# uwoseis/zephyr

Hardware: AMD Instinct MI355X
Metric: wavefields/sec (freq x source solves/s) on 1024^2 grid (higher is better)
Workload: dtype f64

## Files before the change

### include/helm.h

```cpp
#ifndef HELM_H
#define HELM_H

#include <stddef.h>

#ifdef __cplusplus
extern "C" {
#endif

typedef struct helm_op helm_op;

enum { HELM_MINIZEPHYR = 0, HELM_EURUS = 1, HELM_3D = 2  };

enum {
    HELM_BICGSTAB = 0,
    HELM_CGNR = 1,
    HELM_AUTO = 2,
    HELM_MG = 3,
    HELM_DIRECT = 4
};

enum {
    HELM_OK = 0,
    HELM_ERR_ARG = -1,
    HELM_ERR_DEVICE = -2,
// ... 197 lines not shown
    int    pf_prio;
    int    mg3_keep;
    int    mg3_keep_levels;
    int    mg3_galerkin;
    int    mg3_depth_model;
    int    mg3_bt_f32;
    int    mg3_otf;
    int    mg3_f32;
    double mg3_omega;
    int    mg3_coarse;
    int    mg3_nd_leaf;
    int    mg3_bt_twist;
    double mg3_beta;
    double sync_spin_ms;
    int    sync_sleep_us;
    int    nd_fused_sep;
    int    nd_fused_sep_min;
} helm_tuning;
int helm_get_tuning(helm_tuning *out);
int helm_set_tuning(const helm_tuning *t);

int helm_direct_plan(int nz, int nx, int leaf, int *out, int cap);
int helm_direct_plan_front(int nz, int nx, int leaf, int node, long long *cells, int cap);
int helm_debug_zgemm(int device, int M, int N, int K, const double *alpha, const double *A, const double *B,
                     const double *beta, double *C, int batch);
int helm_debug_inverse(int device, int n, double *A, int batch);
int helm_debug_zgemm_bench(int device, int M, int N, int K, int batch, int variant, int reps, double *ms_out);
#define HELM_ZG_TABLE 1
#define HELM_ZG_MASKS 2
#define HELM_ZG_TM64  4
int helm_debug_zgemm_choice(int M, int N, int K, int batch, int nf_div, int force_tile, int force_slab, int have_handle, int mode, int report[5]);
typedef struct helm_zgemm_ex {
    int device, M, N, K, batch;
    int lda, ldb, ldc;
    long long sa, sb, sc;
    double alpha[2], beta[2];
    const double *A; long long a_len;
    double *B; long long b_len;
    double *C; long long c_len;
    int force_tile, force_slab;
    int xcd_map;
    int ntc;
    int zr0, zr1, zc0, zc1, sk0, sk1;
    int tm64, c_is_b;
    const int *tabB, *tabCi, *tabCo; long long tab_len;
    int tab_stride, offB, offCi, offCo;
// ... 53 lines not shown
```

### zephyr_amd/_lib.py

```python
import ctypes
import os
import numpy as np

_HERE = os.path.dirname(os.path.abspath(__file__))
LIB_PATH = os.path.join(_HERE, 'libhelm.so')

HELM_MINIZEPHYR, HELM_EURUS, HELM_3D = 0, 1, 2
HELM_BICGSTAB, HELM_CGNR, HELM_AUTO, HELM_MG, HELM_DIRECT = 0, 1, 2, 3, 4
HELM_RHS_NODE_MAJOR, HELM_OUT_NODE_MAJOR, HELM_NODE_MAJOR = 1, 2, 3
METHODS = {'bicgstab': HELM_BICGSTAB, 'cgnr': HELM_CGNR, 'auto': HELM_AUTO, 'mg': HELM_MG, 'direct': HELM_DIRECT}

ERRORS = {-1: 'HELM_ERR_ARG', -2: 'HELM_ERR_DEVICE', -3: 'HELM_ERR_STATE', -4: 'HELM_ERR_UNSUPPORTED', -5: 'HELM_ERR_PML'}


class HelmError(RuntimeError):
    def __init__(self, code, text):
        self.code = code
        RuntimeError.__init__(self, '%s: %s' % (ERRORS.get(code, code), text))


class SolveOpts(ctypes.Structure):
    _fields_ = [('method', ctypes.c_int), ('rtol', ctypes.c_double), ('maxit', ctypes.c_int),
                ('check_every', ctypes.c_int), ('batch', ctypes.c_int), ('flags', ctypes.c_int)]

# ... 9 lines not shown
                ('factor_ms', ctypes.c_double), ('gemm_ms', ctypes.c_double),
                ('gemm_launches', ctypes.c_longlong), ('gemm_flops', ctypes.c_double),
                ('gemm_big_ms', ctypes.c_double), ('gemm_big_launches', ctypes.c_longlong), ('gemm_big_flops', ctypes.c_double),
                ('gemm_bytes', ctypes.c_double), ('gemm_sol_ms', ctypes.c_double)]


class Tuning(ctypes.Structure):
    _fields_ = [('nd_leaf', ctypes.c_int), ('nd_ws_gb', ctypes.c_double), ('nd_sparse_rhs', ctypes.c_int), ('nd_stable', ctypes.c_int),
                ('nd_stable_thr', ctypes.c_double), ('nd_stable_safety', ctypes.c_double), ('nd_fused_leaf', ctypes.c_int),
                ('nd_fused_leaf_min', ctypes.c_int), ('nd_gjstep', ctypes.c_int), ('nd_gjstep_min', ctypes.c_int), ('nd_overlap', ctypes.c_int),
                ('nd_xcd_map', ctypes.c_int), ('nd_plans', ctypes.c_int), ('nd_direct_out', ctypes.c_int), ('nd_many', ctypes.c_int), ('nd_leaf_idle', ctypes.c_int), ('auto_direct', ctypes.c_int),
                ('auto_mg3', ctypes.c_int), ('prof_ext', ctypes.c_int), ('ws_slots', ctypes.c_int), ('pf_prio', ctypes.c_int),
                ('mg3_keep', ctypes.c_int), ('mg3_keep_levels', ctypes.c_int), ('mg3_galerkin', ctypes.c_int), ('mg3_depth_model', ctypes.c_int),
                ('mg3_bt_f32', ctypes.c_int), ('mg3_otf', ctypes.c_int), ('mg3_f32', ctypes.c_int), ('mg3_omega', ctypes.c_double),
                ('mg3_coarse', ctypes.c_int), ('mg3_nd_leaf', ctypes.c_int), ('mg3_bt_twist', ctypes.c_int), ('mg3_beta', ctypes.c_double), ('sync_spin_ms', ctypes.c_double), ('sync_sleep_us', ctypes.c_int),
                ('nd_fused_sep', ctypes.c_int), ('nd_fused_sep_min', ctypes.c_int)]


class RuntimeStats(ctypes.Structure):
    _fields_ = [('dev_allocs', ctypes.c_longlong), ('dev_alloc_bytes', ctypes.c_double), ('dev_alloc_ms', ctypes.c_double),
                ('host_allocs', ctypes.c_longlong), ('host_alloc_bytes', ctypes.c_double), ('host_alloc_ms', ctypes.c_double),
                ('events_created', ctypes.c_longlong), ('streams_created', ctypes.c_longlong),
                ('first_launches', ctypes.c_longlong), ('first_launch_ms', ctypes.c_double),
                ('kernels_registered', ctypes.c_longlong), ('kernels_resolved', ctypes.c_longlong), ('warm_ms', ctypes.c_double),
                ('dev_frees', ctypes.c_longlong), ('dev_free_ms', ctypes.c_double),
                ('sync_calls', ctypes.c_longlong), ('sync_ms', ctypes.c_double), ('slow_syncs', ctypes.c_longlong), ('worst_sync_ms', ctypes.c_double)]


class ZgemmEx(ctypes.Structure):
    _fields_ = [('device', ctypes.c_int), ('M', ctypes.c_int), ('N', ctypes.c_int), ('K', ctypes.c_int), ('batch', ctypes.c_int),
# ... 125 lines not shown
                                         ctypes.c_void_p, ctypes.c_longlong]),
    'helm_pack_c64_device': (ctypes.c_int, [ctypes.c_void_p, ctypes.c_void_p, ctypes.c_int, ctypes.c_longlong, ctypes.c_void_p, ctypes.c_void_p]),
    'helm_imaging_accumulate_c64_device': (ctypes.c_int, [ctypes.c_void_p, ctypes.c_void_p, ctypes.c_void_p, ctypes.c_void_p, ctypes.c_int,
                                                          ctypes.c_void_p, ctypes.c_void_p]),
    'helm_sample_rows_c64_device': (ctypes.c_int, [ctypes.c_void_p, ctypes.c_void_p, ctypes.c_void_p, ctypes.c_int, ctypes.c_longlong, ctypes.c_void_p,
                                                   ctypes.c_void_p, ctypes.c_void_p, ctypes.c_int, ctypes.c_longlong, ctypes.c_double, ctypes.c_double,
                                                   ctypes.c_double, ctypes.c_double, ctypes.c_void_p]),
    'helm_direct_plan': (ctypes.c_int, [ctypes.c_int, ctypes.c_int, ctypes.c_int, ctypes.c_void_p, ctypes.c_int]),
    'helm_direct_plan_front': (ctypes.c_int, [ctypes.c_int, ctypes.c_int, ctypes.c_int, ctypes.c_int, ctypes.c_void_p, ctypes.c_int]),
    'helm_mg3_axis': (ctypes.c_int, [ctypes.c_int, ctypes.c_int, ctypes.c_double, ctypes.c_double, ctypes.c_double, ctypes.c_double, ctypes.c_int,
                                     ctypes.c_void_p, ctypes.c_void_p, ctypes.c_void_p, ctypes.c_void_p, ctypes.c_void_p, ctypes.c_void_p, ctypes.c_void_p,
                                     ctypes.c_void_p]),
    'helm_debug_zgemm': (ctypes.c_int, [ctypes.c_int, ctypes.c_int, ctypes.c_int, ctypes.c_int, ctypes.c_void_p, ctypes.c_void_p,
                                        ctypes.c_void_p, ctypes.c_void_p, ctypes.c_void_p, ctypes.c_int]),
    'helm_debug_zgemm_choice': (ctypes.c_int, [ctypes.c_int] * 9 + [ctypes.POINTER(ctypes.c_int)]),
    'helm_debug_zgemm_ex': (ctypes.c_int, [ctypes.POINTER(ZgemmEx)]),
    'helm_debug_nm_stage': (ctypes.c_int, [ctypes.c_void_p]),
    'helm_debug_inverse': (ctypes.c_int, [ctypes.c_int, ctypes.c_int, ctypes.c_void_p, ctypes.c_int]),
    'helm_debug_zgemm_bench': (ctypes.c_int, [ctypes.c_int, ctypes.c_int, ctypes.c_int, ctypes.c_int, ctypes.c_int, ctypes.c_int, ctypes.c_int,
                                              ctypes.POINTER(ctypes.c_double)]),
    'helm_set_rhs_support': (ctypes.c_int, [ctypes.c_void_p, ctypes.c_void_p, ctypes.c_longlong, ctypes.c_int]),
    'helm_rhs_support_from_coo': (ctypes.c_int, [ctypes.c_void_p, ctypes.c_void_p, ctypes.c_void_p, ctypes.c_longlong, ctypes.c_void_p, ctypes.c_longlong, ctypes.c_int]),
    'helm_regrid_axis': (ctypes.c_int, [ctypes.c_int, ctypes.c_double, ctypes.c_int, ctypes.c_double, ctypes.c_void_p, ctypes.c_void_p, ctypes.c_int]),
    'helm_regrid_create': (ctypes.c_void_p, [ctypes.c_int, ctypes.c_int, ctypes.c_int, ctypes.c_double, ctypes.c_double, ctypes.c_int, ctypes.c_int,
                                             ctypes.c_double, ctypes.c_double, ctypes.c_double, ctypes.c_double]),
    'helm_regrid_destroy': (None, [ctypes.c_void_p]),
    'helm_regrid_apply_device': (ctypes.c_int, [ctypes.c_void_p, ctypes.c_void_p, ctypes.c_int, ctypes.c_void_p, ctypes.c_longlong, ctypes.c_longlong,
                                                ctypes.c_void_p, ctypes.c_longlong, ctypes.c_longlong, ctypes.c_double, ctypes.c_double, ctypes.c_double,
                                                ctypes.c_void_p]),
    'helm_regrid_apply': (ctypes.c_int, [ctypes.c_void_p, ctypes.c_int, ctypes.c_void_p, ctypes.c_longlong, ctypes.c_longlong, ctypes.c_void_p,
# ... 168 lines not shown
```

### zephyr_amd/csrc/nd_gemm.hip

```cpp
#include "nd_gemm_body.hpp"

thread_local hipEvent_t tl_ev0 = nullptr, tl_ev1 = nullptr;
thread_local int tl_nf_div = 1;
int g_gemm_tile = -1;
int g_gemm_slab = 0;
int g_gemm_xcd = -1;

namespace {

template <int WM, int WN, int MT, int NT, int IDX, int KS, int OCC, int XR = 0>
__global__ __launch_bounds__(256, OCC) void k_zgemm3(int M, int Nn, int K, cplx alpha, const cplx *A0, int lda, long long sa,
                                                     const cplx *B0, int ldb, long long sb, cplx beta, cplx *C0, int ldc, long long sc, GemmRows R) {
    __shared__ cplx tiles[2 * (KS / 4) * (MT * WM + XR + NT * WN) * 64];
    zgemm3_body<WM, WN, MT, NT, IDX, KS, XR>(M, Nn, K, alpha, A0, lda, sa, B0, ldb, sb, beta, C0, ldc, sc, R, tiles);
}

template <int MT, int NT, int KS, int OCC = 2>
void launch_mfma_xr(hipStream_t st, int idx, int nb, int M, int Nn, int K, cplx alpha, const cplx *A, int lda, long long sa, const cplx *B, int ldb, long long sb,
                    cplx beta, cplx *C, int ldc, long long sc, const GemmRows &R) {
    constexpr int TM = 16 * MT + 1, TN = 16 * NT * 4;
    dim3 grid((Nn + TN - 1) / TN, (M + TM - 1) / TM, nb);
    if (idx) ZG_LAUNCH((k_zgemm3<1, 4, MT, NT, 1, KS, OCC, 1>), grid, M, Nn, K, alpha, A, lda, sa, B, ldb, sb, beta, C, ldc, sc, R);
    else ZG_LAUNCH((k_zgemm3<1, 4, MT, NT, 0, KS, OCC, 1>), grid, M, Nn, K, alpha, A, lda, sa, B, ldb, sb, beta, C, ldc, sc, R);
}

template <int WM, int WN, int MT, int NT, int KS, int OCC = 2>
void launch_mfma(hipStream_t st, int idx, int nb, int M, int Nn, int K, cplx alpha, const cplx *A, int lda, long long sa, const cplx *B, int ldb, long long sb,
                 cplx beta, cplx *C, int ldc, long long sc, const GemmRows &R) {
    constexpr int TM = 16 * MT * WM, TN = 16 * NT * WN;
    dim3 grid((Nn + TN - 1) / TN, (M + TM - 1) / TM, nb);
    if (idx == 4) ZG_LAUNCH((k_zgemm3<WM, WN, MT, NT, 4, KS, OCC>), grid, M, Nn, K, alpha, A, lda, sa, B, ldb, sb, beta, C, ldc, sc, R);
    else if (idx == 2) ZG_LAUNCH((k_zgemm3<WM, WN, MT, NT, 2, KS, OCC>), grid, M, Nn, K, alpha, A, lda, sa, B, ldb, sb, beta, C, ldc, sc, R);
    else if (idx) ZG_LAUNCH((k_zgemm3<WM, WN, MT, NT, 1, KS, OCC>), grid, M, Nn, K, alpha, A, lda, sa, B, ldb, sb, beta, C, ldc, sc, R);
    else ZG_LAUNCH((k_zgemm3<WM, WN, MT, NT, 0, KS, OCC>), grid, M, Nn, K, alpha, A, lda, sa, B, ldb, sb, beta, C, ldc, sc, R);
}

constexpr int LBI_KG = 9;
__global__ __launch_bounds__(256, 3) void k_leaf_bwd_idle(int M, int Nn, int K, cplx alpha, const cplx *A0, int lda, long long sa, cplx beta, GemmRows R) {
    constexpr int FA = 4, TMM = 48, TN = 64;
    __shared__ cplx As[LBI_KG * FA * 64];
    int bxi = blockIdx.x, bzi = blockIdx.z;
    if (gridDim.x > 1 && gridDim.z >= 16 && R.xcd_map) {
        const int nt = gridDim.x, nbz = gridDim.z;
        const int L = blockIdx.x + nt * blockIdx.z;
        const int full = (nbz / 8) * 8 * nt;
        if (L < full) { const int grp = L / (8 * nt), w = L % (8 * nt); bzi = grp * 8 + (w & 7); bxi = w >> 3; }
        else { bzi = (nbz / 8) * 8 + (L - full) / nt; bxi = (L - full) % nt; }
    }
    const int n0 = bxi * TN;
// ... 213 lines not shown
    const int dbatch = std::max(1, batch / tl_nf_div);
    if (have_op && !rows && !ext && Nn <= 16 && K >= 1024 && dbatch <= 64) {
        const long long tiles = (long long)dbatch * ((M + 127) / 128);
        if (tiles < 300) {
            ch.ksplit = (int)std::min<long long>(16, std::max<long long>(2, 768 / tiles));
            ch.kc = (((K + ch.ksplit - 1) / ch.ksplit) + 7) & ~7;
        }
    }
    bool latency_mode = false;
    ch.tile = choose_tile(M, Nn, K, dbatch, rows, &latency_mode);
    ch.kslab = latency_mode ? 16 : 8;
    const int idxmode = rows && rows->schur4 ? 4 : (rows && !rows->dense ? (rows->fwd3 ? 2 : 1) : 0);
    const bool plain = !rows || (!rows->schur4 && !rows->fwd3 && !rows->ksplit && rows->zr1 == 0 && rows->zc1 == 0 && rows->sk1 == 0);
    ch.xr = !(rows && rows->la) && M == 49 && Nn >= 64 && plain && idxmode <= 1 && g_gemm_tile < 0;
    if (ch.xr) ch.kslab = 8;
    return ch;
}
void choice_as_split(GemmChoice &ch) { ch.tile = 8; ch.kslab = 8; ch.xr = 0; }

}

int gemm(helm_op *op, int M, int Nn, int K, cplx alpha, const cplx *A, int lda, long long sa, const cplx *B, int ldb, long long sb,
         cplx beta, cplx *C, int ldc, long long sc, int batch, const GemmRows *rows, GemmChoice *made) {
    if (M <= 0 || Nn <= 0 || batch <= 0) return 0;
    hipStream_t st = op ? op->stream : nullptr;
    hipEvent_t e0 = nullptr, e1 = nullptr;
    const bool ext = op && op->profiling && helm_tuning_now().prof_ext != 0;
    const bool in_run = !ext && op && op->gemm_run_depth > 0;
    if (!ext && op && op->profiling && !(in_run && op->gemm_run_pair >= 0)) {
        if (op->ev_used + 2 > op->ev_pool.size() && op->ev_pool.size() < 16384)
            (void)helm_events_grow(op, 64);
        if (op->ev_used + 2 <= op->ev_pool.size()) { e0 = op->ev_pool[op->ev_used]; e1 = op->ev_pool[op->ev_used + 1]; }
    }
// ... 39 lines not shown
            ZG_LAUNCH(k_leaf_bwd_idle, dim3(Nn / 64, 1, nb), M, Nn, K, alpha, Ab, lda, sa, beta, R);
        }
        ExtArm arm(op, ext, 8.0 * M * (double)Nn * K * nb, gemm_operand_bytes(M, Nn, K, beta, rows) * nb, M, Nn, K, nb, idxmode ? idxmode : (rows && rows->la ? 5 : 0));
#define ZG_ARGS st, idxmode, nb, M, Nn, K, alpha, Ab, lda, sa, Bb, ldb, sb, beta, Cb, ldc, sc, R
#define ZG_MFMA(WM_, WN_, MT_, NT_, KS_) launch_mfma<WM_, WN_, MT_, NT_, KS_>(ZG_ARGS)
        if (rows && rows->la) {
            launch_zgemm3_la(st, latency_mode, nb, M, Nn, K, alpha, Ab, lda, sa, Bb, ldb, sb, beta, Cb, ldc, sc, R, *rows->la);
            continue;
        }
        if (ch.xr) { launch_mfma_xr<3, 1, 8>(ZG_ARGS); continue; }
        if (idxmode == 2 && rows->list) {
            ZG_LAUNCH((k_zgemm3<2, 2, 2, 2, 2, 8, 2>), dim3((unsigned)nb * (unsigned)R.nct, (M + 63) / 64, 1), M, Nn, K, alpha, Ab, lda, sa, Bb, ldb, sb, beta, Cb, ldc, sc, R);
            continue;
        }
        if (latency_mode) { if (vsel == 6) ZG_MFMA(2, 2, 1, 1, 16); else ZG_MFMA(1, 4, 1, 1, 16); continue; }
        switch (vsel) {
            case 0: ZG_MFMA(2, 2, 2, 2, 8); break;
            case 1: ZG_MFMA(1, 4, 2, 2, 8); break;
            case 2: ZG_MFMA(1, 4, 1, 4, 8); break;
            case 3: ZG_MFMA(2, 2, 2, 1, 8); break;
            case 4: ZG_MFMA(2, 2, 1, 2, 8); break;
            case 5: ZG_MFMA(1, 4, 1, 2, 8); break;
            case 6: ZG_MFMA(2, 2, 1, 1, 8); break;
            case 8: ZG_MFMA(4, 1, 2, 1, 8); break;
            case 9: ZG_MFMA(2, 2, 4, 2, 8); break;
            default: ZG_MFMA(1, 4, 1, 1, 8); break;
        }
#undef ZG_MFMA
#undef ZG_ARGS
    }
// ... 95 lines not shown
void hook_report(const GemmChoice &ch, int *report) { report[0] = ch.tile; report[1] = ch.kslab; report[2] = ch.xr; report[3] = ch.ksplit; report[4] = ch.kc; }
}

extern "C" int helm_debug_zgemm_choice(int M, int Nn, int K, int batch, int nf_div, int force_tile, int force_slab, int have_handle, int mode, int *report) {
    if (!report || M <= 0 || Nn <= 0 || K <= 0 || batch <= 0 || nf_div < 1 || !hook_force_ok(Nn, force_tile, force_slab) || (mode & ~7)) return HELM_ERR_ARG;
    if ((mode & HELM_ZG_TM64) && M > 64) return HELM_ERR_ARG;
    GemmRows R;
    const GemmRows *rows = hook_rows(mode, R);
    NfDivScope nf(nf_div);
    HookForce force(force_tile, force_slab, -1);
    GemmChoice ch = gemm_choice(have_handle != 0, false, M, Nn, K, batch, rows);
    if (ch.ksplit) choice_as_split(ch);
    hook_report(ch, report);
    return HELM_OK;
}

namespace {
bool zgemm_ex_ok(const helm_zgemm_ex &p) {
    const long long M = p.M, Nn = p.N, K = p.K, nb = p.batch;
    if (M <= 0 || Nn <= 0 || K <= 0 || nb <= 0 || !p.A) return false;
    if (!hook_force_ok(p.N, p.force_tile, p.force_slab) || p.xcd_map < -1 || p.xcd_map > 2) return false;
    const bool table = p.tabB || p.tabCi || p.tabCo;
    if (p.lda < K || p.sa < 0 || (nb - 1) * p.sa + (M - 1) * p.lda + K > p.a_len) return false;
    if (p.c_is_b && (!p.tm64 || p.tabB || p.tabCo || p.C || p.ldc != p.ldb || p.sc != p.sb)) return false;
    if (p.tm64 && M > 64) return false;
    if (!p.tabB) {
        const long long rows = p.c_is_b ? std::max(M, K) : K;
        if (!p.B || p.ldb < Nn || p.sb < 0 || (nb - 1) * p.sb + (rows - 1) * p.ldb + Nn > p.b_len) return false;
        if (p.c_is_b && nb > 1 && p.sb < (rows - 1) * p.ldb + Nn) return false;
    }
// ... 77 lines not shown
    } else R.dense = 1;
    R.zr0 = p.zr0; R.zr1 = p.zr1; R.zc0 = p.zc0; R.zc1 = p.zc1; R.sk0 = p.sk0; R.sk1 = p.sk1;
    R.tm64 = p.tm64; R.ntc = p.ntc ? 1 : 0;
    const GemmRows *rows = (table || masks || p.tm64 || p.ntc) ? &R : nullptr;
    hipError_t e = hipSuccess;
    helm_op *tmp = nullptr;
    if (!bad) {
        const int fs[4] = {0, 0, 0, 0};
        tmp = helm_create(p.device, 0, 8, 8, 1.0, 1.0, 2, fs);
        GemmChoice ch;
        {
            HookForce force(p.force_tile, p.force_slab, p.xcd_map);
            gemm(tmp, p.M, p.N, p.K, cmake(p.alpha[0], p.alpha[1]), dA, p.lda, p.sa, dB, p.ldb, p.sb, cmake(p.beta[0], p.beta[1]), dC, p.ldc, p.sc, p.batch, rows, &ch);
        }
        hook_report(ch, p.report);
        e = hipDeviceSynchronize();
        if (e == hipSuccess) e = hipGetLastError();
        if (e == hipSuccess) {
            if (p.c_is_b) down(p.B, (size_t)p.b_len * 16); else if (p.C) down(p.C, (size_t)p.c_len * 16);
            if (table) { if (p.Cox) down(p.Cox, arena_bytes); if (p.Cox2) down(p.Cox2, arena_bytes); }
            if (dact) hipMemcpy(p.act, dact, (size_t)p.batch * nct * sizeof(int), hipMemcpyDeviceToHost);
        }
    }
    for (auto &d : dev) if (d.second) hipFree(d.second);
    if (tmp) helm_destroy(tmp);
    return (!bad && e == hipSuccess) ? HELM_OK : HELM_ERR_DEVICE;
}

extern "C" int helm_debug_zgemm_bench(int device, int M, int Nn, int K, int batch, int variant, int reps, double *ms_out) {
    helm_tuning_refresh();
// ... 25 lines not shown
```

### zephyr_amd/csrc/nd_gemm_body.hpp

```cpp
#pragma once
#include "nd_internal.hpp"

static __device__ cplx g_zero_page[4];
template <int WM, int WN, int MT, int NT, int IDX, int KS, int XR = 0>
__device__ __forceinline__ void zgemm3_body(int M, int Nn, int K, cplx alpha, const cplx *A0, int lda, long long sa,
                                            const cplx *B0, int ldb, long long sb, cplx beta, cplx *C0, int ldc, long long sc, const GemmRows &R,
                                            cplx *lds) {
    static_assert(WM * WN == 4 && KS % 4 == 0, "four waves per workgroup, k groups of 4");
    static_assert(!XR || (WM == 1 && (IDX == 0 || IDX == 1)), "the extra row needs all four waves side by side and plain / row-table addressing");
    constexpr int TMM = 16 * MT * WM;
    constexpr int TM = TMM + (XR ? 1 : 0), TN = 16 * NT * WN;
    constexpr int FA = TMM / 16 + (XR ? 1 : 0), FB = TN / 16, KG = KS / 4;
    constexpr int NA = (FA * 16 * KS + 255) / 256, NB = (TN * KS + 255) / 256;
    constexpr int XP = 256 / TN;
    constexpr int ABUF = KG * FA * 64, BBUF = KG * FB * 64;
    cplx *As = lds, *Bs = lds + 2 * ABUF;
    __shared__ int kidx[IDX == 1 ? GB_KIDX : 1];
    __shared__ int4 kidx4[IDX == 2 ? GB_KIDX : 1];
    int bxi = blockIdx.x, byi = blockIdx.y, bzi = blockIdx.z;
    if (gridDim.x * gridDim.y > 1 && gridDim.z >= 16 && R.la == nullptr && !(IDX == 0 && R.ksplit > 1) && R.xcd_map && (gridDim.y == 1 || R.xcd_map > 1)) {
        const int nxt = gridDim.x, nt = gridDim.x * gridDim.y, nbz = gridDim.z;
        const int L = blockIdx.x + nxt * blockIdx.y + nt * blockIdx.z;
        const int full = (nbz / 8) * 8 * nt;
        int tile;
// ... 89 lines not shown
        if (nd.kid[0] >= 0) { const NdDev c0 = R.nodes[nd.kid[0]]; ld0 = c0.smax + c0.mmax; S0 = R.arenaS + (long long)R.nf * c0.foff + (long long)kf * c0.mmax * ld0 + c0.smax; base0 = (int)(c0.voff + c0.smax); }
        if (nd.kid[1] >= 0) { const NdDev c1 = R.nodes[nd.kid[1]]; ld1 = c1.smax + c1.mmax; S1 = R.arenaS + (long long)R.nf * c1.foff + (long long)kf * c1.mmax * ld1 + c1.smax; base1 = (int)(c1.voff + c1.smax); }
        for (int t = tid; t < TM + TN; t += 256) {
            const int q = t < TM ? m0 + t : n0 + (t - TM);
            int2 e = make_int2(-1, -1);
            if (q < (t < TM ? M : Nn)) {
                const int4 t4 = R.tabCi[trow + nd.smax + q];
                if (t4.y >= 0 && S0) e.x = t4.y - base0;
                if (t4.z >= 0 && S1) e.y = t4.z - base1;
            }
            if (t < TM) sgr[t] = e; else sgc[t - TM] = e;
        }
        __syncthreads();
    }
    v4f64 cr[MT][NT], ci[MT][NT];
    #pragma unroll
    for (int i = 0; i < MT; ++i)
        #pragma unroll
        for (int j = 0; j < NT; ++j) { cr[i][j] = (v4f64){0, 0, 0, 0}; ci[i][j] = (v4f64){0, 0, 0, 0}; }
    cplx xacc = cmake(0.0, 0.0);
    const int xc = tid % TN, xh = tid / TN;
    cplx ra[NA], rb[NB];
    auto fetch = [&](int k0) {
        #pragma unroll
        for (int e = 0; e < NA; ++e) {
            const int idx = tid + e * 256;
            const int ar = idx / KS, ak = idx % KS;
            cplx v = cmake(0.0, 0.0);
            if (idx < FA * 16 * KS && ar < TM && m0 + ar < M && k0 + ak < K) v = A[(long long)(m0 + ar) * lda + k0 + ak];
            ra[e] = v;
        }
        #pragma unroll
        for (int e = 0; e < NB; ++e) {
            const int idx = tid + e * 256;
// ... 43 lines not shown
    fetch(kbeg);
    stash(0);
    __syncthreads();
    int cur = 0;
    for (int k0 = kbeg; k0 < K; k0 += KS) {
        const bool more = k0 + KS < K;
        if (more) fetch(k0 + KS);
        #pragma unroll
        for (int kg = 0; kg < KG; ++kg) {
            if (KG > 1 && k0 + 4 * kg >= K) break;
            cplx a[MT], b[NT];
            #pragma unroll
            for (int i = 0; i < MT; ++i) a[i] = As[cur * ABUF + (kg * FA + wm * MT + i) * 64 + lq * 16 + (lr ^ lq ^ ((kg & 1) << 2))];
            #pragma unroll
            for (int j = 0; j < NT; ++j) b[j] = Bs[cur * BBUF + (kg * FB + wn * NT + j) * 64 + lane];
            #pragma unroll
            for (int i = 0; i < MT; ++i)
                #pragma unroll
                for (int j = 0; j < NT; ++j) {
                    cr[i][j] = __builtin_amdgcn_mfma_f64_16x16x4f64(a[i].x, b[j].x, cr[i][j], 0, 0, 0);
                    ci[i][j] = __builtin_amdgcn_mfma_f64_16x16x4f64(a[i].x, b[j].y, ci[i][j], 0, 0, 0);
                }
            #pragma unroll
            for (int i = 0; i < MT; ++i) {
                const double nai = -a[i].y;
                #pragma unroll
                for (int j = 0; j < NT; ++j) {
                    cr[i][j] = __builtin_amdgcn_mfma_f64_16x16x4f64(nai, b[j].y, cr[i][j], 0, 0, 0);
                    ci[i][j] = __builtin_amdgcn_mfma_f64_16x16x4f64(a[i].y, b[j].x, ci[i][j], 0, 0, 0);
                }
// ... 81 lines not shown
                    cv[q][j] = cadd(*p0, *p1);
                } else {
                    const cplx *p0 = (ok && cinq[q] && !(cc >= R.zc0 && cc < R.zc1)) ? cinq[q] + cc : g_zero_page;
                    cv[q][j] = *p0;
                }
            }
        #pragma unroll
        for (int q = 0; q < 4; ++q) {
            const int r = m0 + (wm * MT + i) * 16 + lq + 4 * q;
            const bool srow = r >= R.sk0 && r < R.sk1;
            #pragma unroll
            for (int j = 0; j < NT; ++j) {
                const int cc = n0 + (wn * NT + j) * 16 + lr;
                if (!rowok[q] || cc >= Nn || !((colmask >> (((wn * NT + j) * 16 + lr) >> 6)) & 1)) continue;
                if (srow && cc >= R.sk0 && cc < R.sk1) continue;
                cplx v = cmul(alpha, cmake(cr[i][j][q], ci[i][j][q]));
                if (IDX == 4) v = cadd(cv[q][j], v);
                else v = cadd(v, cmul(beta, cv[q][j]));
                if (IDX == 1 && R.cj_out) v = conj_scaled(R.oscale, v);
                if (R.ntc) __builtin_nontemporal_store((v2f64){v.x, v.y}, reinterpret_cast<v2f64 *>(dstq[q] + cc)); else dstq[q][cc] = v;
                if (IDX == 1 && R.Cox2) {
                    const cplx u = conj_scaled(R.oscale, v);
                    __builtin_nontemporal_store((v2f64){u.x, u.y}, reinterpret_cast<v2f64 *>(dstq[q] + (R.Cox2 - R.Cox) + cc));
                }
            }
        }
    }
    if (XR) {
        __syncthreads();
        cplx *part = lds;
        if (xh > 0) part[(xh - 1) * TN + xc] = xacc;
// ... 29 lines not shown
```

### zephyr_amd/csrc/nd_internal.hpp

```cpp
#pragma once
#include "helm_internal.hpp"
#include "direct.hpp"
#include <hip/hip_ext.h>
#include <algorithm>

struct GjPivotArgs { const cplx *T0; int ld; long long stride; int n, k0, nb; const cplx *Wc0, *Wr0; long long wstride; cplx *Pb0; long long pstride; int batch; };
struct GemmRows {
    const int4 *tabB = nullptr, *tabCi = nullptr, *tabCo = nullptr;
    int offB = 0, offCi = 0, offCo = 0, tab_stride = 0;
    const cplx *Bx = nullptr, *Cix = nullptr; cplx *Cox = nullptr;
    int ldx = 0;
    int z0 = 0;
    int fwd3 = 0;
    int zr0 = 0, zr1 = 0, zc0 = 0, zc1 = 0;
    int sk0 = 0, sk1 = 0;
    int ksplit = 0, kc = 0; long long pstride = 0;
    int dense = 0;
    const cplx *Bx2 = nullptr; int k2 = 0;
    int tm64 = 0;
    const GjPivotArgs *la = nullptr;
    int schur4 = 0;
    const NdDev *nodes = nullptr; int first = 0;
    const cplx *arenaS = nullptr;
    int nf = 1;
// ... 125 lines not shown
        double tot = 0;
        for (size_t i = 0; i + 1 < ev.size(); ++i) {
            float ms = 0.f; hipEventElapsedTime(&ms, ev[i], ev[i + 1]); tot += ms;
            const size_t gi = reverse ? P.groups.size() - 1 - i : i;
            if (gi < P.groups.size()) {
                const NdGroup &g = P.groups[gi];
                fprintf(stderr, "[nd trace] %-8s level %2d %s cnt %6d s %5d m %5d : %8.3f ms\n", what, g.level, g.leaf ? "leaf" : "sep ", g.cnt, g.smax, g.mmax, ms);
            } else fprintf(stderr, "[nd trace] %-8s extra : %8.3f ms\n", what, ms);
        }
        fprintf(stderr, "[nd trace] %-8s total %8.3f ms\n", what, tot);
        for (hipEvent_t e : ev) hipEventDestroy(e);
        ev.clear();
    }
};

struct GemmChoice { int tile = 0, kslab = 8, xr = 0, ksplit = 0, kc = 0; };
int gemm(helm_op *op, int M, int Nn, int K, cplx alpha, const cplx *A, int lda, long long sa, const cplx *B, int ldb, long long sb,
         cplx beta, cplx *C, int ldc, long long sc, int batch, const GemmRows *rows = nullptr, GemmChoice *made = nullptr);
extern int g_gemm_tile;
extern int g_gemm_slab;
extern int g_gemm_xcd;
bool gemm_sep_bwd_small(helm_op *op, int smax, int mmax, int nrhs, const cplx *Finv, const cplx *F12, int lda, long long sa, int batch, const GemmRows &rows);
void invert(helm_op *op, cplx *M, int ld, long long stride, int n, int batch, cplx *W, long long ws, int align = 1, int base = 0);
extern int g_recurse_min;
void launch_zgemm3_la(hipStream_t st, bool latency_tile, int nb, int M, int Nn, int K, cplx alpha, const cplx *A, int lda, long long sa, const cplx *B, int ldb, long long sb,
                      cplx beta, cplx *C, int ldc, long long sc, const GemmRows &R, const GjPivotArgs &pv);
void launch_leaf_factor(hipStream_t st, int smax, int nb, const NdDev *d_nodes, int first, cplx *arenaF, cplx *fac, cplx *g21b, const cplx *planes, int nz, int nx, int *flags, int dbg,
                        int nf = 1, int kf = 0);
void launch_sep_factor_small(hipStream_t st, int smax, int nb, const NdDev *d_nodes, int first, cplx *arenaF, cplx *fac, cplx *g21b, const NdPlanesSet &ps, int nz, int nx, int nf,
                             double *est, double *est_rows, long long nbatch_all, int tr);
struct FacSet { int nf = 1; NdFactor *f[ND_NF_MAX] = {nullptr, nullptr, nullptr, nullptr}; const cplx *planes[ND_NF_MAX] = {nullptr, nullptr, nullptr, nullptr}; double rtol[ND_NF_MAX] = {0, 0, 0, 0}; };
// ... 6 lines not shown
```

### zephyr_amd/csrc/runtime.hip

```cpp
#include "helm_internal.hpp"
#include <chrono>
#include <atomic>
#include <unistd.h>
#include <time.h>
#include <mutex>
#include <thread>
#include <map>
#include <cstring>
#include <algorithm>

namespace {
struct KernelRec { const void *fn; const char *pretty; std::atomic<bool> launched{false}; };
struct KernelRegistry {
    std::mutex mu;
    std::vector<KernelRec *> recs;
    std::atomic<KernelRec *> fast[2048];
    std::atomic<int> n{0};
};
KernelRegistry &kreg() { static KernelRegistry *r = new KernelRegistry(); return *r; }
struct RuntimeCounters {
    std::atomic<long long> dev_frees{0}, dev_free_us{0}, sync_calls{0}, sync_us{0}, slow_syncs{0}, worst_sync_us{0};
    std::atomic<long long> dev_allocs{0}, dev_alloc_bytes{0}, dev_alloc_us{0}, host_allocs{0}, host_alloc_bytes{0}, host_alloc_us{0},
                           events{0}, streams{0}, first_launches{0}, first_launch_us{0}, resolved{0}, warm_us{0};
};
// ... 171 lines not shown
    t.nd_stable_safety = std::max(1.0, t.nd_stable_safety);
    if (!(t.nd_stable_thr >= 0)) t.nd_stable_thr = 0.0;
    t.nd_fused_leaf_min = std::max(1, t.nd_fused_leaf_min);
    t.nd_gjstep_min = std::max(64, t.nd_gjstep_min);
    t.nd_plans = std::max(1, t.nd_plans);
    t.ws_slots = std::min(4, std::max(1, t.ws_slots));
    t.pf_prio = t.pf_prio > 0 ? 1 : (t.pf_prio < 0 ? -1 : 0);
    if (!(t.mg3_omega > 0) || t.mg3_omega > 2.0) t.mg3_omega = 0.9;
    t.mg3_coarse = std::min(2, std::max(0, t.mg3_coarse));
    t.mg3_nd_leaf = std::max(2, t.mg3_nd_leaf);
    if (!std::isfinite(t.mg3_beta) || t.mg3_beta < 0) t.mg3_beta = 0.0;
    if (!(t.sync_spin_ms >= 0)) t.sync_spin_ms = 0.0;
    t.sync_spin_ms = std::min(t.sync_spin_ms, 60000.0);
    t.sync_sleep_us = std::min(100000, std::max(0, t.sync_sleep_us));
    t.nd_fused_sep_min = std::max(1, t.nd_fused_sep_min);
}
static helm_tuning tuning_from_env() {
    helm_tuning t;
    t.nd_leaf = helm_env_int("HELM_ND_LEAF", 8);
    t.nd_ws_gb = tune_d("HELM_ND_WS_GB", 32.0);
    t.nd_sparse_rhs = helm_env_int("HELM_ND_SPARSE_RHS", 1);
    t.nd_stable = helm_env_int("HELM_ND_STABLE", 1);
    t.nd_stable_thr = tune_d("HELM_ND_STABLE_THR", 0.0);
    t.nd_stable_safety = tune_d("HELM_ND_STABLE_SAFETY", 8.0);
    t.nd_fused_leaf = helm_env_int("HELM_ND_FUSEDLEAF", 1);
    t.nd_fused_leaf_min = helm_env_int("HELM_ND_FUSEDLEAF_MIN", 2048);
    t.nd_gjstep = helm_env_int("HELM_ND_GJSTEP", 1);
    t.nd_gjstep_min = helm_env_int("HELM_ND_GJSTEP_MIN", 128);
    t.nd_overlap = helm_env_int("HELM_ND_OVERLAP_NM", 1);
    t.nd_xcd_map = helm_env_int("HELM_ND_XCDMAP", 2);
// ... 8 lines not shown
    t.pf_prio = helm_env_int("HELM_PF_PRIO", 1);
    t.mg3_keep = helm_env_int("HELM_MG3_KEEP", 1);
    t.mg3_keep_levels = helm_env_int("HELM_MG3_KEEP_LEVELS", -1);
    t.mg3_galerkin = helm_env_int("HELM_MG3_GALERKIN", 1);
    t.mg3_depth_model = helm_env_int("HELM_MG3_DEPTH_MODEL", 1);
    t.mg3_bt_f32 = helm_env_int("HELM_MG3_BT_F32", 1);
    t.mg3_otf = helm_env_int("HELM_MG3_OTF", 1);
    t.mg3_f32 = helm_env_int("HELM_MG3_F32", 1);
    t.mg3_omega = tune_d("HELM_MG3_OMEGA", 0.9);
    { const char *cs = getenv("HELM_MG3_COARSE"); t.mg3_coarse = cs && !strcmp(cs, "nd") ? 1 : (cs && !strcmp(cs, "bt") ? 2 : 0); }
    t.mg3_nd_leaf = helm_env_int("HELM_MG3_ND_LEAF", 2);
    t.mg3_bt_twist = helm_env_int("HELM_MG3_BT_TWIST", 1);
    t.mg3_beta = tune_d("HELM_MG3_BETA", 0.0);
    t.sync_spin_ms = tune_d("HELM_SYNC_SPIN_MS", 0.0);
    t.sync_sleep_us = helm_env_int("HELM_SYNC_SLEEP_US", 0);
    t.nd_fused_sep = helm_env_int("HELM_ND_FUSEDSEP", 1);
    t.nd_fused_sep_min = helm_env_int("HELM_ND_FUSEDSEP_MIN", 512);
    tuning_clamp(t);
    return t;
}
extern char **environ;
static unsigned long long env_fingerprint() {
    unsigned long long h = 1469598103934665603ull;
    for (char **e = environ; e && *e; ++e) {
        const char *s = *e;
        if (s[0] != 'H' || s[1] != 'E' || s[2] != 'L' || s[3] != 'M' || s[4] != '_') continue;
        for (; *s; ++s) { h ^= (unsigned char)*s; h *= 1099511628211ull; }
        h ^= 0xff; h *= 1099511628211ull;
    }
    return h;
// ... 542 lines not shown
```

Baseline: 15940.

## Use 3M (Gauss) complex multiply in MFMA zgemm for compute-bound shapes

Adds a 3M variant of the f64 MFMA complex GEMM kernel. It accumulates Ar*Br, Ai*Bi and (Ar+Ai)(Br+Bi) with three MFMAs instead of four, then recombines them into real and imaginary parts in the epilogue. A roofline-style heuristic enables it by default for large-K, large-M dense or gather products that are estimated to be compute-bound. This trades one MFMA per k-step for an extra accumulator set, which raises register pressure, and for slightly different rounding in the imaginary part.

Result: slower. 14750 (-7.5%).

```diff
diff --git a/include/helm.h b/include/helm.h
--- a/include/helm.h
+++ b/include/helm.h
@@ -235,6 +235,9 @@
     double mg3_beta;
     double sync_spin_ms;
     int    sync_sleep_us;
+    int    nd_gemm3m;
+    int    nd_gemm3m_min_k;
+    int    nd_gemm3m_min_rows;
     int    nd_fused_sep;
     int    nd_fused_sep_min;
 } helm_tuning;
@@ -251,6 +254,11 @@
 #define HELM_ZG_MASKS 2
 #define HELM_ZG_TM64  4
 int helm_debug_zgemm_choice(int M, int N, int K, int batch, int nf_div, int force_tile, int force_slab, int have_handle, int mode, int report[5]);
+#define HELM_ZG3M_LA    8
+#define HELM_ZG3M_MASKS 16
+#define HELM_ZG3M_TM64  32
+int helm_debug_zgemm_3m(int M, int N, int K, int batch, int nf_div, int mode, int out[4]);
+long long helm_debug_zgemm_3m_launches(void);
 typedef struct helm_zgemm_ex {
     int device, M, N, K, batch;
     int lda, ldb, ldc;
diff --git a/zephyr_amd/_lib.py b/zephyr_amd/_lib.py
--- a/zephyr_amd/_lib.py
+++ b/zephyr_amd/_lib.py
@@ -47,6 +47,7 @@
                 ('mg3_keep', ctypes.c_int), ('mg3_keep_levels', ctypes.c_int), ('mg3_galerkin', ctypes.c_int), ('mg3_depth_model', ctypes.c_int),
                 ('mg3_bt_f32', ctypes.c_int), ('mg3_otf', ctypes.c_int), ('mg3_f32', ctypes.c_int), ('mg3_omega', ctypes.c_double),
                 ('mg3_coarse', ctypes.c_int), ('mg3_nd_leaf', ctypes.c_int), ('mg3_bt_twist', ctypes.c_int), ('mg3_beta', ctypes.c_double), ('sync_spin_ms', ctypes.c_double), ('sync_sleep_us', ctypes.c_int),
+                ('nd_gemm3m', ctypes.c_int), ('nd_gemm3m_min_k', ctypes.c_int), ('nd_gemm3m_min_rows', ctypes.c_int),
                 ('nd_fused_sep', ctypes.c_int), ('nd_fused_sep_min', ctypes.c_int)]
 
 
@@ -202,6 +203,8 @@
     'helm_debug_zgemm': (ctypes.c_int, [ctypes.c_int, ctypes.c_int, ctypes.c_int, ctypes.c_int, ctypes.c_void_p, ctypes.c_void_p,
                                         ctypes.c_void_p, ctypes.c_void_p, ctypes.c_void_p, ctypes.c_int]),
     'helm_debug_zgemm_choice': (ctypes.c_int, [ctypes.c_int] * 9 + [ctypes.POINTER(ctypes.c_int)]),
+    'helm_debug_zgemm_3m': (ctypes.c_int, [ctypes.c_int] * 6 + [ctypes.POINTER(ctypes.c_int)]),
+    'helm_debug_zgemm_3m_launches': (ctypes.c_longlong, []),
     'helm_debug_zgemm_ex': (ctypes.c_int, [ctypes.POINTER(ZgemmEx)]),
     'helm_debug_nm_stage': (ctypes.c_int, [ctypes.c_void_p]),
     'helm_debug_inverse': (ctypes.c_int, [ctypes.c_int, ctypes.c_int, ctypes.c_void_p, ctypes.c_int]),
diff --git a/zephyr_amd/csrc/nd_gemm.hip b/zephyr_amd/csrc/nd_gemm.hip
--- a/zephyr_amd/csrc/nd_gemm.hip
+++ b/zephyr_amd/csrc/nd_gemm.hip
@@ -1,18 +1,21 @@
 #include "nd_gemm_body.hpp"
+#include <atomic>
 
 thread_local hipEvent_t tl_ev0 = nullptr, tl_ev1 = nullptr;
 thread_local int tl_nf_div = 1;
 int g_gemm_tile = -1;
 int g_gemm_slab = 0;
 int g_gemm_xcd = -1;
+static std::atomic<long long> g_gemm3m_launches{0};
+static int g_gemm3m_last_ex = -1;
 
 namespace {
 
-template <int WM, int WN, int MT, int NT, int IDX, int KS, int OCC, int XR = 0>
+template <int WM, int WN, int MT, int NT, int IDX, int KS, int OCC, int XR = 0, int M3 = 0>
 __global__ __launch_bounds__(256, OCC) void k_zgemm3(int M, int Nn, int K, cplx alpha, const cplx *A0, int lda, long long sa,
                                                      const cplx *B0, int ldb, long long sb, cplx beta, cplx *C0, int ldc, long long sc, GemmRows R) {
     __shared__ cplx tiles[2 * (KS / 4) * (MT * WM + XR + NT * WN) * 64];
-    zgemm3_body<WM, WN, MT, NT, IDX, KS, XR>(M, Nn, K, alpha, A0, lda, sa, B0, ldb, sb, beta, C0, ldc, sc, R, tiles);
+    zgemm3_body<WM, WN, MT, NT, IDX, KS, XR, M3>(M, Nn, K, alpha, A0, lda, sa, B0, ldb, sb, beta, C0, ldc, sc, R, tiles);
 }
 
 template <int MT, int NT, int KS, int OCC = 2>
@@ -33,6 +36,17 @@
     else if (idx == 2) ZG_LAUNCH((k_zgemm3<WM, WN, MT, NT, 2, KS, OCC>), grid, M, Nn, K, alpha, A, lda, sa, B, ldb, sb, beta, C, ldc, sc, R);
     else if (idx) ZG_LAUNCH((k_zgemm3<WM, WN, MT, NT, 1, KS, OCC>), grid, M, Nn, K, alpha, A, lda, sa, B, ldb, sb, beta, C, ldc, sc, R);
     else ZG_LAUNCH((k_zgemm3<WM, WN, MT, NT, 0, KS, OCC>), grid, M, Nn, K, alpha, A, lda, sa, B, ldb, sb, beta, C, ldc, sc, R);
+}
+
+template <int WM, int WN, int MT, int NT, int KS, int OCC = 2>
+void launch_mfma_3m(hipStream_t st, int idx, int nb, int M, int Nn, int K, cplx alpha, const cplx *A, int lda, long long sa, const cplx *B, int ldb, long long sb,
+                    cplx beta, cplx *C, int ldc, long long sc, const GemmRows &R) {
+    constexpr int TM = 16 * MT * WM, TN = 16 * NT * WN;
+    dim3 grid((Nn + TN - 1) / TN, (M + TM - 1) / TM, nb);
+    if (idx == 4) ZG_LAUNCH((k_zgemm3<WM, WN, MT, NT, 4, KS, 3, 0, 1>), grid, M, Nn, K, alpha, A, lda, sa, B, ldb, sb, beta, C, ldc, sc, R);
+    else if (idx) ZG_LAUNCH((k_zgemm3<WM, WN, MT, NT, 1, KS, OCC, 0, 1>), grid, M, Nn, K, alpha, A, lda, sa, B, ldb, sb, beta, C, ldc, sc, R);
+    else ZG_LAUNCH((k_zgemm3<WM, WN, MT, NT, 0, KS, OCC, 0, 1>), grid, M, Nn, K, alpha, A, lda, sa, B, ldb, sb, beta, C, ldc, sc, R);
+    g_gemm3m_launches.fetch_add(1, std::memory_order_relaxed);
 }
 
 constexpr int LBI_KG = 9;
@@ -276,9 +290,16 @@
     const bool plain = !rows || (!rows->schur4 && !rows->fwd3 && !rows->ksplit && rows->zr1 == 0 && rows->zc1 == 0 && rows->sk1 == 0);
     ch.xr = !(rows && rows->la) && M == 49 && Nn >= 64 && plain && idxmode <= 1 && g_gemm_tile < 0;
     if (ch.xr) ch.kslab = 8;
+    const helm_tuning tune = helm_tuning_now();
+    const bool m3_shape = (ch.tile == 0 || ch.tile == 1) && !latency_mode && !ch.ksplit && !ch.xr && !(rows && rows->la) && idxmode != 2;
+    if (m3_shape && tune.nd_gemm3m >= 2) ch.m3 = 1;
+    else if (m3_shape && tune.nd_gemm3m == 1 && g_gemm_tile < 0 && K >= tune.nd_gemm3m_min_k && M >= tune.nd_gemm3m_min_rows) {
+        const double fl = 8.0 * M * (double)Nn * K, by = gemm_operand_bytes(M, Nn, K, cmake(1.0, 0.0), rows);
+        ch.m3 = fl / 78.6e12 > by / 8.0e12 ? 1 : 0;
+    }
     return ch;
 }
-void choice_as_split(GemmChoice &ch) { ch.tile = 8; ch.kslab = 8; ch.xr = 0; }
+void choice_as_split(GemmChoice &ch) { ch.tile = 8; ch.kslab = 8; ch.xr = 0; ch.m3 = 0; }
 
 }
 
@@ -348,6 +369,7 @@
             continue;
         }
         if (latency_mode) { if (vsel == 6) ZG_MFMA(2, 2, 1, 1, 16); else ZG_MFMA(1, 4, 1, 1, 16); continue; }
+        if (ch.m3) { if (vsel == 0) launch_mfma_3m<2, 2, 2, 2, 8>(ZG_ARGS); else launch_mfma_3m<1, 4, 2, 2, 8>(ZG_ARGS); continue; }
         switch (vsel) {
             case 0: ZG_MFMA(2, 2, 2, 2, 8); break;
             case 1: ZG_MFMA(1, 4, 2, 2, 8); break;
@@ -473,6 +495,31 @@
     hook_report(ch, report);
     return HELM_OK;
 }
+
+extern "C" int helm_debug_zgemm_3m(int M, int Nn, int K, int batch, int nf_div, int mode, int *out) {
+    const int addr = mode & 7, force = mode >> 8;
+    if (!out || M <= 0 || Nn <= 0 || K <= 0 || batch <= 0 || nf_div < 1 || mode < 0 || !(addr == 0 || addr == 1 || addr == 2 || addr == 4) || force > 9 ||
+        (force && !hook_force_ok(Nn, force - 1, 0))) return HELM_ERR_ARG;
+    if ((mode & HELM_ZG3M_TM64) && M > 64) return HELM_ERR_ARG;
+    helm_tuning_refresh();
+    GemmRows R;
+    GjPivotArgs pv{};
+    const GemmRows *rows = nullptr;
+    if (addr || (mode & (HELM_ZG3M_LA | HELM_ZG3M_MASKS | HELM_ZG3M_TM64))) {
+        rows = &R;
+        R.dense = addr == 0; R.fwd3 = addr == 2; R.schur4 = addr == 4;
+        if (mode & HELM_ZG3M_LA) R.la = &pv;
+        if (mode & HELM_ZG3M_MASKS) R.zr1 = 1;
+        if (mode & HELM_ZG3M_TM64) R.tm64 = 1;
+    }
+    NfDivScope nf(nf_div);
+    HookForce frc(force ? force - 1 : -1, 0, -1);
+    GemmChoice ch = gemm_choice(true, false, M, Nn, K, batch, rows);
+    if (ch.ksplit) choice_as_split(ch);
+    out[0] = ch.m3; out[1] = g_gemm3m_last_ex; out[2] = ch.tile; out[3] = ch.kslab;
+    return HELM_OK;
+}
+extern "C" long long helm_debug_zgemm_3m_launches(void) { return g_gemm3m_launches.load(std::memory_order_relaxed); }
 
 namespace {
 bool zgemm_ex_ok(const helm_zgemm_ex &p) {
@@ -580,6 +627,7 @@
             gemm(tmp, p.M, p.N, p.K, cmake(p.alpha[0], p.alpha[1]), dA, p.lda, p.sa, dB, p.ldb, p.sb, cmake(p.beta[0], p.beta[1]), dC, p.ldc, p.sc, p.batch, rows, &ch);
         }
         hook_report(ch, p.report);
+        g_gemm3m_last_ex = ch.m3;
         e = hipDeviceSynchronize();
         if (e == hipSuccess) e = hipGetLastError();
         if (e == hipSuccess) {
diff --git a/zephyr_amd/csrc/nd_gemm_body.hpp b/zephyr_amd/csrc/nd_gemm_body.hpp
--- a/zephyr_amd/csrc/nd_gemm_body.hpp
+++ b/zephyr_amd/csrc/nd_gemm_body.hpp
@@ -2,12 +2,13 @@
 #include "nd_internal.hpp"
 
 static __device__ cplx g_zero_page[4];
-template <int WM, int WN, int MT, int NT, int IDX, int KS, int XR = 0>
+template <int WM, int WN, int MT, int NT, int IDX, int KS, int XR = 0, int M3 = 0>
 __device__ __forceinline__ void zgemm3_body(int M, int Nn, int K, cplx alpha, const cplx *A0, int lda, long long sa,
                                             const cplx *B0, int ldb, long long sb, cplx beta, cplx *C0, int ldc, long long sc, const GemmRows &R,
                                             cplx *lds) {
     static_assert(WM * WN == 4 && KS % 4 == 0, "four waves per workgroup, k groups of 4");
     static_assert(!XR || (WM == 1 && (IDX == 0 || IDX == 1)), "the extra row needs all four waves side by side and plain / row-table addressing");
+    static_assert(!M3 || (!XR && IDX != 2), "the 3M form exists for the dense, row-table and Schur-gather products of the full tiles");
     constexpr int TMM = 16 * MT * WM;
     constexpr int TM = TMM + (XR ? 1 : 0), TN = 16 * NT * WN;
     constexpr int FA = TMM / 16 + (XR ? 1 : 0), FB = TN / 16, KG = KS / 4;
@@ -127,10 +128,11 @@
         __syncthreads();
     }
     v4f64 cr[MT][NT], ci[MT][NT];
+    v4f64 ct[M3 ? MT : 1][M3 ? NT : 1];
     #pragma unroll
     for (int i = 0; i < MT; ++i)
         #pragma unroll
-        for (int j = 0; j < NT; ++j) { cr[i][j] = (v4f64){0, 0, 0, 0}; ci[i][j] = (v4f64){0, 0, 0, 0}; }
+        for (int j = 0; j < NT; ++j) { cr[i][j] = (v4f64){0, 0, 0, 0}; ci[i][j] = (v4f64){0, 0, 0, 0}; if (M3) ct[M3 ? i : 0][M3 ? j : 0] = (v4f64){0, 0, 0, 0}; }
     cplx xacc = cmake(0.0, 0.0);
     const int xc = tid % TN, xh = tid / TN;
     cplx ra[NA], rb[NB];
@@ -204,6 +206,22 @@
             for (int i = 0; i < MT; ++i) a[i] = As[cur * ABUF + (kg * FA + wm * MT + i) * 64 + lq * 16 + (lr ^ lq ^ ((kg & 1) << 2))];
             #pragma unroll
             for (int j = 0; j < NT; ++j) b[j] = Bs[cur * BBUF + (kg * FB + wn * NT + j) * 64 + lane];
+            if (M3) {
+                double as[MT], bs[NT];
+                #pragma unroll
+                for (int i = 0; i < MT; ++i) as[i] = a[i].x + a[i].y;
+                #pragma unroll
+                for (int j = 0; j < NT; ++j) bs[j] = b[j].x + b[j].y;
+                #pragma unroll
+                for (int i = 0; i < MT; ++i)
+                    #pragma unroll
+                    for (int j = 0; j < NT; ++j) {
+                        cr[i][j] = __builtin_amdgcn_mfma_f64_16x16x4f64(a[i].x, b[j].x, cr[i][j], 0, 0, 0);
+                        ci[i][j] = __builtin_amdgcn_mfma_f64_16x16x4f64(a[i].y, b[j].y, ci[i][j], 0, 0, 0);
+                        ct[M3 ? i : 0][M3 ? j : 0] = __builtin_amdgcn_mfma_f64_16x16x4f64(as[i], bs[j], ct[M3 ? i : 0][M3 ? j : 0], 0, 0, 0);
+                    }
+                continue;
+            }
             #pragma unroll
             for (int i = 0; i < MT; ++i)
                 #pragma unroll
@@ -315,7 +333,8 @@
                 const int cc = n0 + (wn * NT + j) * 16 + lr;
                 if (!rowok[q] || cc >= Nn || !((colmask >> (((wn * NT + j) * 16 + lr) >> 6)) & 1)) continue;
                 if (srow && cc >= R.sk0 && cc < R.sk1) continue;
-                cplx v = cmul(alpha, cmake(cr[i][j][q], ci[i][j][q]));
+                const cplx acc = M3 ? cmake(cr[i][j][q] - ci[i][j][q], (ct[M3 ? i : 0][M3 ? j : 0][q] - cr[i][j][q]) - ci[i][j][q]) : cmake(cr[i][j][q], ci[i][j][q]);
+                cplx v = cmul(alpha, acc);
                 if (IDX == 4) v = cadd(cv[q][j], v);
                 else v = cadd(v, cmul(beta, cv[q][j]));
                 if (IDX == 1 && R.cj_out) v = conj_scaled(R.oscale, v);
diff --git a/zephyr_amd/csrc/nd_internal.hpp b/zephyr_amd/csrc/nd_internal.hpp
--- a/zephyr_amd/csrc/nd_internal.hpp
+++ b/zephyr_amd/csrc/nd_internal.hpp
@@ -163,7 +163,7 @@
     }
 };
 
-struct GemmChoice { int tile = 0, kslab = 8, xr = 0, ksplit = 0, kc = 0; };
+struct GemmChoice { int tile = 0, kslab = 8, xr = 0, ksplit = 0, kc = 0, m3 = 0; };
 int gemm(helm_op *op, int M, int Nn, int K, cplx alpha, const cplx *A, int lda, long long sa, const cplx *B, int ldb, long long sb,
          cplx beta, cplx *C, int ldc, long long sc, int batch, const GemmRows *rows = nullptr, GemmChoice *made = nullptr);
 extern int g_gemm_tile;
diff --git a/zephyr_amd/csrc/runtime.hip b/zephyr_amd/csrc/runtime.hip
--- a/zephyr_amd/csrc/runtime.hip
+++ b/zephyr_amd/csrc/runtime.hip
@@ -209,6 +209,9 @@
     t.sync_spin_ms = std::min(t.sync_spin_ms, 60000.0);
     t.sync_sleep_us = std::min(100000, std::max(0, t.sync_sleep_us));
     t.nd_fused_sep_min = std::max(1, t.nd_fused_sep_min);
+    t.nd_gemm3m = std::min(2, std::max(0, t.nd_gemm3m));
+    t.nd_gemm3m_min_k = std::max(1, t.nd_gemm3m_min_k);
+    t.nd_gemm3m_min_rows = std::max(1, t.nd_gemm3m_min_rows);
 }
 static helm_tuning tuning_from_env() {
     helm_tuning t;
@@ -247,6 +250,9 @@
     t.mg3_beta = tune_d("HELM_MG3_BETA", 0.0);
     t.sync_spin_ms = tune_d("HELM_SYNC_SPIN_MS", 0.0);
     t.sync_sleep_us = helm_env_int("HELM_SYNC_SLEEP_US", 0);
+    t.nd_gemm3m = helm_env_int("HELM_ND_GEMM3M", 1);
+    t.nd_gemm3m_min_k = helm_env_int("HELM_ND_GEMM3M_MIN_K", 64);
+    t.nd_gemm3m_min_rows = helm_env_int("HELM_ND_GEMM3M_MIN_ROWS", 128);
     t.nd_fused_sep = helm_env_int("HELM_ND_FUSEDSEP", 1);
     t.nd_fused_sep_min = helm_env_int("HELM_ND_FUSEDSEP_MIN", 512);
     tuning_clamp(t);
```
